# drwangxian/viterbi_spl

Hardware: AMD Instinct MI355X
Metric: Viterbi Mframes/s at S=361 T=30k; achieved HBM GB/s vs peak (higher is better)
Workload: dtype f32

## Files before the change

viterbi_spl_amd/csrc/banded.hip:

```cpp
#include "device_common.hpp"

namespace vit {

template <int W, int NWT, bool DW, bool DBG, int NXT, typename ET>
__global__ void __launch_bounds__((NWT + (DW ? 3 : 2)) * 64) banded_forward_kernel(FwdArgs a) {
    extern __shared__ __align__(16) unsigned char smem[];
    constexpr int NP = NWT * 64;
    constexpr int EPL = NWT;
    const int S = a.S, SP = a.SP, T = a.T, SD = a.SD;
    constexpr int DC = NP + 16;
    float* dls = reinterpret_cast<float*>(smem);
    float* dl = dls + 4;
    float* Pv = dls + 4 * DC;
    float* Sv = Pv + NP + 1;
    float* Dv = Sv + NP + 1;
    VI* tot = reinterpret_cast<VI*>(Dv + kMaxDenseRows);

    const int tid = threadIdx.x;
    const int lane = tid & 63;
    const int wv = __builtin_amdgcn_readfirstlane(tid >> 6);
    const int song = blockIdx.x;
    const int Tb = song_length(a.lengths, song, T);
    const ET* __restrict__ E = reinterpret_cast<const ET*>(a.logE) + (size_t)song * T * S;
    float* __restrict__ hist = a.hist + (size_t)song * T * SD;
// ... 259 lines not shown
    }
    const int sh = a.win_shift;
    const int lov = (tvalid ? lo : S - W) + sh;
    const float* rp = dls + 4 + (lov & 3) * DC + (lov & ~3) + 16 * hh;
    constexpr bool XS = XQ;
    float* fmp = fmg + (XS ? split_fm_slot(lane, is_x) : fm_slot(lane));
    static_assert(!XQ || NXT == 1, "the extra column leaves M by address only where the launcher proved its quad idle");

    for (int k = tid; k < L::reset; k += NW * 64) dls[k] = -INFINITY;
    __syncthreads();

#ifdef VIT_TIMING_HOOKS
    const bool probe = (a.debug & 48) != 0;
    constexpr bool wprobe = WPR;
    WaveProbe wp_;
#else
    constexpr bool probe = false;
#endif
    unsigned long long clk0 = 0ull, rt0 = 0ull;

    auto body = [&](auto role, auto resets) {
        constexpr bool HALF = decltype(role)::value, RESETS = decltype(resets)::value;
        constexpr int WL = HALF ? W / 2 : WF;
        constexpr bool TRIM = WL % 4 != 0;
        const float cj = own ? reinterpret_cast<const float*>(a.image + a.off_rowc)[jc] : -INFINITY;
        float aw[WL];
        float xa[NXL > 0 ? NXL : 1];
        {
            const float* __restrict__ tab = reinterpret_cast<const float*>(a.image + a.off_tabA);
            const float* __restrict__ xaT = reinterpret_cast<const float*>(a.image + a.off_extraA);
#pragma unroll
            for (int w = 0; w < WL; ++w) aw[w] = tvalid ? tab[(size_t)(w + (HALF ? 16 * hh : 0)) * SP + jc] : -INFINITY;
#pragma unroll
            for (int k = 0; k < NXL; ++k)
                xa[k] = (tvalid && k < nx && (!HALF || hh == 1)) ? xaT[(size_t)k * SP + jc] : -INFINITY;
        }
        [[maybe_unused]] float* wp = nullptr;
        if constexpr (HALF) wp = dls + 4 + sh + j + hh * split_upper_off(DC);
        else {
            static_assert(L::dls == 0 && DC == kSplitCopyStride && BUF == 4 * DC, "split_addtid_base / split_addtid_imm (plan.hpp) speak of this layout");
            static_assert(split_addtid_imm(1, 3) + split_addtid_base(3, NWF - 1) + 4 * 64 <= (int)L::bytes() && L::bytes() < 65536,
                          "the largest immediate, the largest base and their sum with the lane term: inside the segment, hence 16 bits each");
            lds_addtid_base(reinterpret_cast<const float*>(smem + split_addtid_base(sh, wv)));
        }
        [[maybe_unused]] int xo[NXL > 0 ? NXL : 1];
        if constexpr (!XS) {
#pragma unroll
            for (int k = 0; k < NXL; ++k) {
                xo[k] = 4 + sh + xcol[k];
                asm volatile("" : "+v"(xo[k]));
            }
        }

        auto produce = [&](const float dn, auto wbc, const int G, const int Z) {
            constexpr int WB = decltype(wbc)::value;
            if constexpr (HALF) {
#pragma unroll
                for (int c = 0; c < 2; ++c) wp[WB * BUF + floor_copy_off(DC, c)] = dn;
            } else {
                split_frames(std::make_integer_sequence<int, 4>{}, [&](auto cc) {
                    static_assert(split_addtid_imm(WB, decltype(cc)::value) == 4 * (WB * BUF + floor_copy_off(DC, decltype(cc)::value)), "the ds_write_b32 form's offset");
                    lds_store_addtid<split_addtid_imm(WB, decltype(cc)::value)>(dn);
                });
            }
            fm_publish(fmp + G * kFmGroupFloats, (!XQ && NXL > 0 && is_x) ? -INFINITY : dn);
            if constexpr (RESETS) fmg[Z * kFmGroupFloats + lane] = -INFINITY;
        };

        {
            const float d0 = tvalid ? reinterpret_cast<const float*>(a.image + a.off_logpi)[j] + load_e<ET>(E + j) : -INFINITY;
            if (own) hist[j] = d0;
            produce(d0, std::integral_constant<int, 0>{}, 0, 1);
        }
        auto frame_barrier = [&] {
            if constexpr (!HALF) __builtin_amdgcn_s_waitcnt(split_waitcnt(kNoVmWait, 0));
            __syncthreads();
        };
        float er[PF];
#pragma unroll
        for (int k = 0; k < PF; ++k) er[k] = load_e<ET>(E + (size_t)(1 + k < Tb ? 1 + k : Tb - 1) * S + jld);
#pragma unroll
        for (int w = 0; w < WL; ++w) asm volatile("" ::"v"(aw[w]));
#pragma unroll
        for (int k = 0; k < NXL; ++k) asm volatile("" ::"v"(xa[k]));
        asm volatile("" ::"v"(cj));
        frame_barrier();

        const unsigned rowH = 4u * (unsigned)SD, rowE = (unsigned)sizeof(ET) * (unsigned)S;
        float* hb = hist;
        const ET* eb = E;
        unsigned elim = 0;
        auto round_bases = [&](const int t) {
            const int r = split_prefetch_row(t, 0, PF, Tb, false);
            const int ahead = Tb - 1 - r < PF ? Tb - 1 - r : PF;
            hb = hist + (size_t)(t - 1) * SD;
            eb = E + (size_t)r * S;
            elim = (unsigned)ahead * rowE;
        };
        auto interior_bases = [&](const int t) {
            hb = hist + (size_t)(t - 1) * SD;
            eb = E + (size_t)split_prefetch_row(t, 0, PF, Tb, true) * S;
        };
        auto frame = [&](float& e_slot, auto uc, auto ic) {
            constexpr int u = decltype(uc)::value;
            constexpr bool INTERIOR = decltype(ic)::value;
            constexpr int RB = u & 1, WB = RB ^ 1;
            const int GR = u % kFmGroups, GW = (u + 1) % kFmGroups, GZ = (u + 2) % kFmGroups;
            const f32x4* __restrict__ win = reinterpret_cast<const f32x4*>(rp + RB * BUF);
            float xd[NXL > 0 ? NXL : 1];
            f32x4 fq;
            [[maybe_unused]] float m0, m1 = -INFINITY, m2 = -INFINITY, m3 = -INFINITY;
            if constexpr (!XS) {
#pragma unroll
                for (int k = 0; k < NXL; ++k) xd[k] = dls[xo[k] + RB * BUF];
            }
            fq = reinterpret_cast<const f32x4*>(fmg + GR * kFmGroupFloats)[0];
            asm volatile("" ::: "memory");
            f32x4 dw[WL / 4];
#pragma unroll
            for (int q = 0; q < WL / 4; ++q) dw[q] = win[q];
            [[maybe_unused]] float ds = 0.f;
            if constexpr (TRIM) ds = (rp + RB * BUF)[WL - 1];
            __builtin_amdgcn_sched_barrier(0);
#ifdef VIT_TIMING_HOOKS
            if constexpr (wprobe && !TRIM) wp_.first_data(fq);
#endif
            if constexpr (TRIM) {
                static_assert(split_reads_behind(WL / 4, 0) == WL / 4 + 1 - 2, "behind the first pair: every other window read of the burst");
                __builtin_amdgcn_s_waitcnt(split_waitcnt(kNoVmWait, split_reads_behind(WL / 4, 0)));
                asm volatile("" : "+v"(fq), "+v"(dw[0]), "+v"(dw[1]));
#ifdef VIT_TIMING_HOOKS
                if constexpr (wprobe) wp_.first_data(fq);
#endif
            }
            const float M = XS ? fmaxf(fmaxf(fq.x, fq.y), fq.z) : fmaxf(fmaxf(fq.x, fq.y), fmaxf(fq.z, fq.w));
            if constexpr (XS) xd[0] = fq.w;
            m0 = M + cj;
            asm volatile("" ::"v"(m0));
            __builtin_amdgcn_sched_barrier(0);
            float mx;
            constexpr int vmw = PF - 1 + u;
            static_assert(vmw <= 2 * (PF - 1) && 2 * (PF - 1) < kNoVmWait, "vmcnt bound: one store and one load per frame, 6-bit field");
            if constexpr (TRIM) {
                constexpr int NQ = WL / 4, TQ = NQ % 2 ? 1 : 2, NPB = (NQ - TQ) / 2;
                static_assert(NXL == 1 && NQ >= 3 && 2 * NPB + TQ == NQ && 4 * NQ + 1 == WL, "pairs of quads, then the tail: one or two quads and one float");
                static_assert(split_reads_behind(NQ, 0) <= 15, "lgkmcnt is a four-bit field");
                static_assert(split_reads_behind(NQ, NPB - 1) == TQ + 1, "behind the last pair stand the tail's reads -- TQ quads and the float -- and nothing else");
                static_assert(split_reads_behind(NQ, NPB) + 2 == TQ + 1 && TQ <= 2, "the tail's wait, lgkmcnt(0), leaves no window read out");
                float mb = xd[0] + xa[0];
                asm volatile("" ::"v"(mb));
                split_frames(std::make_integer_sequence<int, NPB>{}, [&](auto gc) {
                    constexpr int w = 8 * decltype(gc)::value;
                    f32x4 da = dw[w / 4], db = dw[w / 4 + 1];
                    if constexpr (decltype(gc)::value >= 1) {
                        constexpr int behind = split_reads_behind(NQ, decltype(gc)::value);
                        static_assert(behind >= TQ + 1 && behind + 2 == split_reads_behind(NQ, decltype(gc)::value - 1), "two reads fewer than the pair before");
                        __builtin_amdgcn_s_waitcnt(split_waitcnt(kNoVmWait, behind));
                        asm volatile("" : "+v"(da), "+v"(db));
                    }
                    f32x2 c0_ = f32x2{da.x, da.y} + f32x2{aw[w + 0], aw[w + 1]};
                    f32x2 c1_ = f32x2{da.z, da.w} + f32x2{aw[w + 2], aw[w + 3]};
                    f32x2 c2_ = f32x2{db.x, db.y} + f32x2{aw[w + 4], aw[w + 5]};
                    f32x2 c3_ = f32x2{db.z, db.w} + f32x2{aw[w + 6], aw[w + 7]};
                    asm volatile("" : "+v"(c0_), "+v"(c1_), "+v"(c2_), "+v"(c3_));
                    m0 = fmaxf(fmaxf(m0, c0_.x), c0_.y);
                    mb = fmaxf(fmaxf(mb, c1_.x), c1_.y);
                    m0 = fmaxf(fmaxf(m0, c2_.x), c2_.y);
                    mb = fmaxf(fmaxf(mb, c3_.x), c3_.y);
                });
                {
                    constexpr int w = 8 * NPB;
                    f32x4 da = dw[w / 4], db = dw[NQ - 1];
                    __builtin_amdgcn_s_waitcnt(split_waitcnt(vmw, 0));
                    if constexpr (TQ == 2) asm volatile("" : "+v"(da), "+v"(db), "+v"(ds)); else asm volatile("" : "+v"(da), "+v"(ds));
                    f32x2 c0_ = f32x2{da.x, da.y} + f32x2{aw[w + 0], aw[w + 1]};
                    f32x2 c1_ = f32x2{da.z, da.w} + f32x2{aw[w + 2], aw[w + 3]};
                    float cs = ds + aw[WL - 1];
                    if constexpr (TQ == 2) {
                        f32x2 c2_ = f32x2{db.x, db.y} + f32x2{aw[w + 4], aw[w + 5]};
                        f32x2 c3_ = f32x2{db.z, db.w} + f32x2{aw[w + 6], aw[w + 7]};
                        asm volatile("" : "+v"(c0_), "+v"(c1_), "+v"(c2_), "+v"(c3_), "+v"(cs));
                        m0 = fmaxf(fmaxf(m0, c0_.x), c0_.y);
                        mb = fmaxf(fmaxf(mb, c1_.x), c1_.y);
                        m0 = fmaxf(fmaxf(m0, c2_.x), c2_.y);
                        mb = fmaxf(fmaxf(mb, c3_.x), c3_.y);
                    } else {
                        asm volatile("" : "+v"(c0_), "+v"(c1_), "+v"(cs));
                        m0 = fmaxf(fmaxf(m0, c0_.x), c0_.y);
                        mb = fmaxf(fmaxf(mb, c1_.x), c1_.y);
                    }
                    mx = fmaxf(fmaxf(m0, mb), cs);
                }
            } else {
                split_frames(std::make_integer_sequence<int, WL / 8>{}, [&](auto gc) {
                    constexpr int w = 8 * decltype(gc)::value;
                    constexpr bool last = w + 8 == WL;
                    constexpr bool pairw = w + 16 >= WL && w >= 8;
                    f32x4 da = dw[w / 4], db = dw[w / 4 + 1];
                    if constexpr (pairw) {
                        __builtin_amdgcn_s_waitcnt(split_waitcnt(last ? vmw : kNoVmWait, last ? 0 : 2));
                        asm volatile("" : "+v"(da), "+v"(db));
                    }
                    f32x2 c0_ = f32x2{da.x, da.y} + f32x2{aw[w + 0], aw[w + 1]};
                    f32x2 c1_ = f32x2{da.z, da.w} + f32x2{aw[w + 2], aw[w + 3]};
                    f32x2 c2_ = f32x2{db.x, db.y} + f32x2{aw[w + 4], aw[w + 5]};
                    f32x2 c3_ = f32x2{db.z, db.w} + f32x2{aw[w + 6], aw[w + 7]};
                    asm volatile("" : "+v"(c0_), "+v"(c1_), "+v"(c2_), "+v"(c3_));
                    m0 = fmaxf(fmaxf(m0, c0_.x), c0_.y);
                    m1 = fmaxf(fmaxf(m1, c1_.x), c1_.y);
                    m2 = fmaxf(fmaxf(m2, c2_.x), c2_.y);
                    m3 = fmaxf(fmaxf(m3, c3_.x), c3_.y);
                });
#pragma unroll
                for (int k = 0; k < NXL; ++k) m1 = fmaxf(m1, xd[k] + xa[k]);
                mx = fmaxf(fmaxf(m0, m1), fmaxf(m2, m3));
            }
            if constexpr (HALF) mx = max_lane_xor8(mx);
            const float dn = mx + e_slot;
#ifdef VIT_TIMING_HOOKS
            if constexpr (wprobe) wp_.before_publish(dn);
#endif
            const float sv = (HALF && is_fm) ? M : dn;
            const unsigned eso = INTERIOR ? (unsigned)u * rowE : ((unsigned)u * rowE < elim ? (unsigned)u * rowE : elim);
            produce(dn, std::integral_constant<int, WB>{}, GW, GZ);
            asm volatile("" ::: "memory");
            row_store_f32(hb, hoffb, sv, (unsigned)u * rowH);
            e_slot = row_load_e<ET>(eb, eoffb, eso);
#ifdef VIT_TIMING_HOOKS
            if constexpr (wprobe) wp_.barrier(); else
#endif
            frame_barrier();
        };
#ifdef VIT_TIMING_HOOKS
        if constexpr (wprobe) wp_.start();
#endif
        clk0 = probe ? __builtin_amdgcn_s_memtime() : 0ull;
        rt0 = probe ? __builtin_amdgcn_s_memrealtime() : 0ull;
        if constexpr (HALF) __builtin_amdgcn_s_setprio(1);
        int t = 1;
        for (; split_round_interior(t, PF, Tb); t += PF) {
// ... 363 lines not shown
```

viterbi_spl_amd/csrc/banded_floor.inc:

```
__device__ __forceinline__ __amdgpu_buffer_rsrc_t row_rsrc(const void* row) {
    return __builtin_amdgcn_make_buffer_rsrc(const_cast<void*>(row), (short)0, -1, 0x00020000);
}
__device__ __forceinline__ void row_store_f32(float* row, unsigned off, float v, unsigned soff = 0) {
    __builtin_amdgcn_raw_buffer_store_b32(__float_as_uint(v), row_rsrc(row), off, soff, 0);
}
template <typename ET>
__device__ __forceinline__ float row_load_e(const ET* row, unsigned off, unsigned soff = 0);
template <>
__device__ __forceinline__ float row_load_e<float>(const float* row, unsigned off, unsigned soff) {
    return __uint_as_float(__builtin_amdgcn_raw_buffer_load_b32(row_rsrc(row), off, soff, 0));
}
template <>
__device__ __forceinline__ float row_load_e<__half>(const __half* row, unsigned off, unsigned soff) {
    return __half2float(__ushort_as_half(__builtin_amdgcn_raw_buffer_load_b16(row_rsrc(row), off, soff, 0)));
}

inline constexpr int kFmGroups = 4;
inline constexpr int kFmGroupFloats = 64;
inline constexpr int kFmSlots = 4;
__device__ __forceinline__ int fm_slot(int lane) { return 4 * (lane & 3) + ((lane >> 2) & 3); }
__device__ __forceinline__ void fm_publish(float* slot, float v) {
    v = fmaxf(v, __int_as_float(__builtin_amdgcn_update_dpp(0, __float_as_int(v), 0xb1, 0xf, 0xf, false)));
    v = fmaxf(v, __int_as_float(__builtin_amdgcn_update_dpp(0, __float_as_int(v), 0x4e, 0xf, 0xf, false)));
    __hip_atomic_fetch_max(slot, v, __ATOMIC_RELAXED, __HIP_MEMORY_SCOPE_WORKGROUP);
// ... 2 lines not shown
#ifdef VIT_TIMING_HOOKS
struct WaveProbe {
    unsigned long long t_rel = 0, t_pub = 0, t_dat = 0, work = 0, wait = 0, data = 0;
    __device__ __forceinline__ void start() { t_rel = t_dat = __builtin_amdgcn_s_memtime(); }
    template <typename V>
    __device__ __forceinline__ void first_data(V& first) {
        asm volatile("" : "+v"(first));
        __builtin_amdgcn_sched_barrier(0);
        t_dat = __builtin_amdgcn_s_memtime();
        __builtin_amdgcn_sched_barrier(0);
    }
    __device__ __forceinline__ void before_publish(float dn) {
        __builtin_amdgcn_sched_barrier(0);
        asm volatile("" ::"v"(dn));
        t_pub = __builtin_amdgcn_s_memtime();
        __builtin_amdgcn_sched_barrier(0);
    }
    __device__ __forceinline__ void barrier() {
        unsigned long long t_in, t_out;
        asm volatile("s_waitcnt lgkmcnt(0)\n\ts_memtime %0\n\ts_barrier\n\ts_memtime %1\n\ts_waitcnt lgkmcnt(0)"
                     : "=&s"(t_in), "=&s"(t_out) : "s"(t_pub), "s"(t_dat) : "memory");
        work += t_pub - t_rel;
        data += t_dat - t_rel;
        wait += t_out - t_in;
        t_rel = t_dat = t_out;
    }
    __device__ __forceinline__ void finish(float* scratch, int wv, int lane, int frames) const {
        if (lane != 0) return;
        const float n = (float)(frames > 0 ? frames : 1);
        scratch[4 * wv + 0] = (float)__builtin_amdgcn_s_getreg((1 << 11) | (4 << 6) | 4);
        scratch[4 * wv + 1] = (float)work / n;
        scratch[4 * wv + 2] = (float)wait / n;
        scratch[4 * wv + 3] = n;
        scratch[48 + wv] = (float)data / n;
    }
};
#endif

template <int W, int NWT, WgVariant V = WgVariant::Plain>
struct FloorLds {
    static constexpr int NP = NWT * 64;
    static constexpr int DC = NP + 16;
    static constexpr int BUF = 4 * DC;
    static constexpr int WR = (W == 128 && NWT > 8) ? (V != WgVariant::Plain ? 88 : 96) : W;
    static constexpr int dls = 0;
    static constexpr int fmg = dls + 2 * BUF;
    static constexpr int reset = fmg + kFmGroups * kFmGroupFloats;
    static constexpr int tot = reset;
    static constexpr int awl = tot + 16 * (int)(sizeof(VI) / sizeof(float));
    static constexpr int end = awl + (W - WR) / 4 * 4 * NP;
    static_assert(sizeof(float) * end <= kLdsBytes, "one workgroup's LDS");
    static constexpr size_t bytes() { return sizeof(float) * end; }
};
constexpr int floor_copy_off(int DC, int c) { return c * DC - c; }
constexpr int split_upper_off(int DC) { return floor_copy_off(DC, 2); }
inline constexpr int kSplitFullWaves = 4, kSplitHalfWaves = 4;
inline constexpr int kSplitStates = 64 * kSplitFullWaves + 32 * kSplitHalfWaves;
using FloorSplitLds = FloorLds<32, kSplitStates / 64>;
constexpr int split_half_of(int lane) { return (lane >> 3) & 1; }
constexpr int split_half_target(int lane) { return ((lane >> 4) << 3) | (lane & 7); }
inline constexpr int kSplitXSlot = 3;
constexpr int split_fm_slot(int lane, bool is_x) { return 4 * (lane & 3) + (is_x ? kSplitXSlot : (lane >> 2) % 3); }

template <int W, int NWT, int NXT, int PF, typename ET, WgVariant V = WgVariant::Plain, bool WPR = false>
__global__ void __launch_bounds__(NWT * 64) banded_floor_forward_kernel(FwdArgs a) {
    static_assert(!WPR || V == WgVariant::Plain, "the per-wave probe exists for the plain kernel only");
    using L = FloorLds<W, NWT, V>;
    constexpr bool PK = V == WgVariant::Packed, CK = V == WgVariant::Ckpt, PC = V == WgVariant::PackedCkpt;
    constexpr bool PKx = PK || PC;
    constexpr bool CKx = CK || PC;
    extern __shared__ __align__(16) unsigned char smem[];
    constexpr int NP = L::NP, DC = L::DC, BUF = L::BUF, WR = L::WR;
    float* dls = reinterpret_cast<float*>(smem) + L::dls;
    float* fmg = dls + L::fmg;
    VI* tot = reinterpret_cast<VI*>(dls + L::tot);
    f32x4* awl = reinterpret_cast<f32x4*>(dls + L::awl);
    const int S = a.S, SP = a.SP, T = a.T, SD = a.SD;
    constexpr bool GEN = NXT < 0;
    constexpr int NXL = GEN ? kMaxExtras : NXT;
    const int nx = GEN ? a.n_extras : NXT;

    const int tid = threadIdx.x;
    const int lane = tid & 63;
    const int wv = __builtin_amdgcn_readfirstlane(tid >> 6);
    constexpr int kPast = 1, kRowBias = 1;
#define VIT_WG_CURSOR 1
#include "wg_cursor.inc"
#define VIT_WG_CURSOR 2
#include "wg_cursor.inc"

    const int j = tid;
    const bool tvalid = j < S;
    const int jc = tvalid ? j : 0;
    const int jld = tvalid ? j : S - 1;
    const unsigned hoff = tvalid ? (unsigned)(SD + j) : ((j == S && !(CKx && ck_every > 0)) ? (unsigned)S : (unsigned)(SD + S + 1));
    const bool is_fm = j == S;
    const unsigned hoffb = 4u * hoff, eoffb = (unsigned)(sizeof(ET) * jld);
    const int lo = reinterpret_cast<const int32_t*>(a.image + a.off_lo)[jc];
    const float cj = tvalid ? reinterpret_cast<const float*>(a.image + a.off_rowc)[jc] : -INFINITY;
    float aw[WR];
    float xa[NXL > 0 ? NXL : 1];
    int xcol[NXL > 0 ? NXL : 1];
    bool is_x = false;
    {
        const float* __restrict__ tab = reinterpret_cast<const float*>(a.image + a.off_tabA);
        const float* __restrict__ xaT = reinterpret_cast<const float*>(a.image + a.off_extraA);
#pragma unroll
        for (int w = 0; w < WR; ++w) aw[w] = tvalid ? tab[(size_t)w * SP + jc] : -INFINITY;
#pragma unroll
        for (int q = 0; q < (W - WR) / 4; ++q) {
            f32x4 wv4;
            wv4.x = tvalid ? tab[(size_t)(WR + 4 * q + 0) * SP + jc] : -INFINITY;
            wv4.y = tvalid ? tab[(size_t)(WR + 4 * q + 1) * SP + jc] : -INFINITY;
            wv4.z = tvalid ? tab[(size_t)(WR + 4 * q + 2) * SP + jc] : -INFINITY;
            wv4.w = tvalid ? tab[(size_t)(WR + 4 * q + 3) * SP + jc] : -INFINITY;
// ... 255 lines not shown
```

viterbi_spl_amd/csrc/device_common.hpp:

```cpp
#pragma once
#include <hip/hip_fp16.h>
#include <hip/hip_runtime.h>

#include <cstddef>
#include <cstdint>
#include <type_traits>

#include "kernels.hpp"

namespace vit {

inline constexpr int kBig = 0x7fffffff;
inline constexpr size_t kLdsBytes = 160 * 1024;

typedef float f32x2 __attribute__((ext_vector_type(2)));
typedef float f32x4 __attribute__((ext_vector_type(4)));
typedef float f32x4_u __attribute__((ext_vector_type(4), aligned(4)));
typedef float f32x2_u __attribute__((ext_vector_type(2), aligned(4)));
typedef int i32x4_u __attribute__((ext_vector_type(4), aligned(4)));
typedef _Float16 f16x2_u __attribute__((ext_vector_type(2), aligned(2)));
typedef _Float16 f16x4_u __attribute__((ext_vector_type(4), aligned(2)));

__device__ __forceinline__ int song_length(const int64_t* lengths, int song, int T) {
    if (!lengths) return T;
// ... 27 lines not shown
        "s_nop 1\n\t"
        "v_max_f32_dpp %0, %0, %0 row_bcast:15 row_mask:0xa bank_mask:0xf\n\t"
        "s_nop 1\n\t"
        "v_max_f32_dpp %0, %0, %0 row_bcast:31 row_mask:0xc bank_mask:0xf\n\t"
        "s_nop 1"
        : "+v"(x));
    return x;
}
__device__ __forceinline__ float wave_max_all(float x) {
    return __int_as_float(__builtin_amdgcn_readlane(__float_as_int(wave_scan_max(x)), 63));
}
template <int CTRL, int ROW_MASK>
__device__ __forceinline__ double dpp_max_step_f64(const double x) {
    const long long b = __double_as_longlong(x);
    const int lo = (int)(unsigned)(b & 0xffffffffll), hi = (int)(b >> 32);
    const int slo = __builtin_amdgcn_update_dpp(lo, lo, CTRL, ROW_MASK, 0xf, false);
    const int shi = __builtin_amdgcn_update_dpp(hi, hi, CTRL, ROW_MASK, 0xf, false);
    const double s = __longlong_as_double(((long long)shi << 32) | (long long)(unsigned)slo);
    return fmax(x, s);
}
__device__ __forceinline__ double wave_scan_max_f64(double x) {
    x = dpp_max_step_f64<0x111, 0xf>(x);
    x = dpp_max_step_f64<0x112, 0xf>(x);
    x = dpp_max_step_f64<0x114, 0xf>(x);
    x = dpp_max_step_f64<0x118, 0xf>(x);
    x = dpp_max_step_f64<0x142, 0xa>(x);
    x = dpp_max_step_f64<0x143, 0xc>(x);
    return x;
}
__device__ __forceinline__ double readlane_f64(const double x, const int l) {
    const long long b = __double_as_longlong(x);
    const unsigned lo = (unsigned)__builtin_amdgcn_readlane((int)(unsigned)(b & 0xffffffffll), l);
    const unsigned hi = (unsigned)__builtin_amdgcn_readlane((int)(b >> 32), l);
    return __longlong_as_double((long long)(((unsigned long long)hi << 32) | lo));
}
__device__ __forceinline__ double wave_max_all_f64(const double x) { return readlane_f64(wave_scan_max_f64(x), 63); }
__device__ __forceinline__ float max_other_half(float x) {
    const auto r = __builtin_amdgcn_permlane32_swap(__float_as_uint(x), __float_as_uint(x), false, false);
    return fmaxf(__uint_as_float(r[0]), __uint_as_float(r[1]));
}
inline constexpr int kDppRowRor8 = 0x128;
__device__ __forceinline__ float max_lane_xor8(float x) {
    return fmaxf(x, __int_as_float(__builtin_amdgcn_update_dpp(0, __float_as_int(x), kDppRowRor8, 0xf, 0xf, false)));
}
__device__ __forceinline__ void lds_addtid_base(const float* p) {
    const unsigned base = (unsigned)(unsigned long)(__attribute__((address_space(3))) const float*)p;
    asm volatile("s_mov_b32 m0, %0\n\ts_nop 0" ::"s"(base) : "memory");
}
template <int BYTE_OFF>
__device__ __forceinline__ void lds_store_addtid(float v) {
    static_assert(BYTE_OFF >= 0 && BYTE_OFF < 65536 && BYTE_OFF % 4 == 0, "the instruction's 16-bit offset field");
    asm volatile("ds_write_addtid_b32 %0 offset:%1" ::"v"(v), "n"(BYTE_OFF) : "memory");
}
__device__ __forceinline__ float wave_shift_up(float x, float fill) {
    return __int_as_float(__builtin_amdgcn_update_dpp(__float_as_int(fill), __float_as_int(x), 0x138, 0xf, 0xf, false));
}
__device__ __forceinline__ float wave_shift_down(float x, float fill) {
    return __int_as_float(__builtin_amdgcn_update_dpp(__float_as_int(fill), __float_as_int(x), 0x130, 0xf, 0xf, false));
}
__device__ __forceinline__ float dpp_shr1(float x) {
    return __int_as_float(__builtin_amdgcn_update_dpp(0, __float_as_int(x), 0x138, 0xf, 0xf, true));
}
__device__ __forceinline__ float dpp_shl1(float x) {
    return __int_as_float(__builtin_amdgcn_update_dpp(0, __float_as_int(x), 0x130, 0xf, 0xf, true));
}

struct VI {
    float v;
    int i;
};

__device__ __forceinline__ VI vi_identity() { return VI{-INFINITY, kBig}; }
__device__ __forceinline__ VI op_fwd(VI earlier, VI later) { return later.v > earlier.v ? later : earlier; }
__device__ __forceinline__ VI op_rev(VI acc, VI next) { return next.v >= acc.v ? next : acc; }

template <int CTRL, int ROW_MASK>
__device__ __forceinline__ VI dpp_fetch(VI x) {
    VI r;
    r.v = __int_as_float(__builtin_amdgcn_update_dpp(__float_as_int(-INFINITY), __float_as_int(x.v), CTRL,
                                                     ROW_MASK, 0xf, false));
    r.i = __builtin_amdgcn_update_dpp(kBig, x.i, CTRL, ROW_MASK, 0xf, false);
    return r;
}

template <bool REV>
__device__ __forceinline__ VI wave_scan(VI x) {
#define VIT_SCAN_STEP(CTRL, MASK)                        \
    {                                                    \
        VI s = dpp_fetch<CTRL, MASK>(x);                 \
        x = REV ? op_rev(s, x) : op_fwd(s, x);           \
    }
    VIT_SCAN_STEP(0x111, 0xf)
    VIT_SCAN_STEP(0x112, 0xf)
    VIT_SCAN_STEP(0x114, 0xf)
    VIT_SCAN_STEP(0x118, 0xf)
    VIT_SCAN_STEP(0x142, 0xa)
    VIT_SCAN_STEP(0x143, 0xc)
#undef VIT_SCAN_STEP
    return x;
}

__device__ __forceinline__ void terminal_argmax(float dj, int j, bool valid, VI* tot, int nw, int32_t* last_state,
                                                float* loglik, int song) {
    VI x{valid ? dj : -INFINITY, valid ? j : kBig};
    x = wave_scan<false>(x);
    if ((threadIdx.x & 63) == 63) tot[threadIdx.x >> 6] = x;
// ... 27 lines not shown
```

viterbi_spl_amd/csrc/floor_lds_check.hip:

```cpp
#include <cstdio>
#include <cstdlib>
#include <vector>

#include "device_common.hpp"

namespace vit {
#include "banded_floor.inc"
}
using namespace vit;

static int failures = 0;
#define CHECK(cond, ...)                                                     \
    do {                                                                     \
        if (!(cond)) {                                                       \
            if (++failures <= 20) { std::printf("FAIL %s: ", #cond); std::printf(__VA_ARGS__); std::printf("\n"); } \
        }                                                                    \
    } while (0)

static bool write2_encodable(int stride) { return stride >= 0 && stride <= 255; }
static bool write2st64_encodable(int stride) { return stride >= 0 && stride % 64 == 0 && stride / 64 <= 255; }

struct Segment {
    std::vector<int> owner;
    explicit Segment(int n) : owner((size_t)n, -1) {}
// ... 151 lines not shown
            was[hw] = half_wave_read_cycles(S, off, sh, hw, old_half_of, old_half_target);
            now[hw] = half_wave_read_cycles(S, off, sh, hw, split_half_of, split_half_target);
            if (sh == off % 4) CHECK(now[hw] <= was[hw], "S %d sh %d half wave %d: %d LDS cycles for its window reads, %d with the halves 32 lanes apart", S, sh, hw, now[hw], was[hw]);
        }
        std::printf("split window reads S %d off %d sh %d%s: ds_read_b128 cycles per half wave, halves 32 lanes apart %d / %d / %d / %d, partner l ^ 8 %d / %d / %d / %d\n",
                    S, off, sh, sh == off % 4 ? " (the plan's)" : "", was[0], was[1], was[2], was[3], now[0], now[1], now[2], now[3]);
    }
}

static void replay_slot_map() {
    int cases = 0;
    for (int S = 64 * kSplitFullWaves + 1; S < kSplitStates; S += 4) {
        const int x = S - 1;
        CHECK(x % 4 == 0, "x %d", x);
        bool x_reached = false;
        for (int wv = 0; wv < kSplitFullWaves + kSplitHalfWaves; ++wv) {
            bool quad_in_m[16] = {};
            for (int lane = 0; lane < 64; ++lane) {
                const bool half = wv >= kSplitFullWaves;
                const int j = half ? 64 * kSplitFullWaves + 32 * (wv - kSplitFullWaves) + split_half_target(lane) : 64 * wv + lane;
                const int slot = split_fm_slot(lane, j == x);
                CHECK(slot >= 0 && slot < 16, "slot %d", slot);
                bool quad_has_x = false;
                for (int m = 0; m < 4; ++m) {
                    const int lm = (lane & ~3) | m;
                    const int jm = half ? 64 * kSplitFullWaves + 32 * (wv - kSplitFullWaves) + split_half_target(lm) : 64 * wv + lm;
                    quad_has_x |= jm == x;
                    if (quad_has_x && jm != x) CHECK(jm >= S, "S %d: state %d shares a quad with x and is live", S, jm);
                }
                if (slot < kSplitXSlot) {
                    CHECK(!quad_has_x, "S %d wave %d lane %d: a quad that holds x adds into M slot %d", S, wv, lane, slot);
                    quad_in_m[lane >> 2] = true;
                }
                if (slot == kSplitXSlot) {
                    CHECK(j == x, "S %d wave %d lane %d (state %d) adds into the extra column's slot", S, wv, lane, j);
                    x_reached = true;
                }
            }
            for (int q = 0; q < 16; ++q) {
                bool has_x = false;
                for (int m = 0; m < 4; ++m) {
                    const int lm = 4 * q + m;
                    has_x |= (wv >= kSplitFullWaves ? 64 * kSplitFullWaves + 32 * (wv - kSplitFullWaves) + split_half_target(lm) : 64 * wv + lm) == x;
                }
                CHECK(quad_in_m[q] != has_x, "S %d wave %d quad %d: %s", S, wv, q, has_x ? "holds x and reaches M" : "reaches none of slots 0 .. 2");
            }
        }
        CHECK(x_reached, "S %d: no lane adds x into slot %d", S, kSplitXSlot);
        ++cases;
    }
    std::printf("split slot map: every quad without x reaches one of slots 0 .. 2, x reaches slot %d alone: ok (%d state counts)\n", kSplitXSlot, cases);
}

template <int W, int NWT>
static void replay_pair() {
    char name[64];
    std::snprintf(name, sizeof name, "FloorLds<%d, %d>", W, NWT);
    replay<FloorLds<W, NWT, WgVariant::Plain>, W>(name, NWT, false);
    if constexpr (W == 128 && NWT > 8) {
        std::snprintf(name, sizeof name, "FloorLds<%d, %d, Packed>", W, NWT);
        replay<FloorLds<W, NWT, WgVariant::Packed>, W>(name, NWT, false);
    }
}
template <int W>
static void replay_width() {
    replay_pair<W, 2>();
    replay_pair<W, 4>();
    replay_pair<W, 6>();
    replay_pair<W, 8>();
    replay_pair<W, 12>();
}

int main() {
    static_assert(sizeof(kBandedWidths) / sizeof(int) == 6, "one call per instantiated window width");
    replay_width<16>();
    replay_width<32>();
    replay_width<64>();
    replay_width<84>();
    replay_width<96>();
    replay_width<128>();
    replay<FloorSplitLds, 32>("FloorSplitLds (split kernel)", kSplitStates / 64, true);
    replay_lane_map();
    replay_slot_map();
    replay_read_cycles(361, 15);
    replay_read_cycles(321, 13);
    static_assert(2 * FloorSplitLds::bytes() <= kLdsBytes && 2 * FloorLds<32, 6>::bytes() <= kLdsBytes, "two workgroups share a CU's LDS");
    if (failures) { std::printf("%d check(s) failed\n", failures); return 1; }
    std::printf("floor LDS layouts: all checks passed\n");
    return 0;
}
```

viterbi_spl_amd/csrc/plan.hpp:

```cpp
#pragma once
#include <cstddef>
#include <cstdint>
#include <vector>

namespace vit {

constexpr int kMaxExtras = 4;
constexpr int kMaxDenseRows = 4;
inline constexpr int kBandedWidths[] = {16, 32, 64, 84, 96, 128};
constexpr bool banded_width_instantiated(int W) {
    for (int w : kBandedWidths)
        if (w == W) return true;
    return false;
}

struct BandedPlan {
    bool ok = false;
    int S = 0;
    int SP = 0;
    float c0 = 0.f;
    std::vector<float> rowc;
    int n_extras = 0;
    int extras[kMaxExtras] = {0, 0, 0, 0};
    int n_dense = 0;
// ... 3 lines not shown
    std::vector<int32_t> lo;
    std::vector<int32_t> kind;
    bool lo_affine = false;
    bool floor_ok = false;
    std::vector<int32_t> live_last;
    bool pair_ok = false;
    std::vector<int32_t> lo2;
    bool lo2_affine = false;
    int lo2_off = 0;
    int lo_off = 0;

    bool step_ok = false;
    int step_bw = 0, step_kb = 0;
    std::vector<float> stepC;
    float step_cn = 0.f;

    bool floor_all_ok = false;
    bool wave_ok = false;
    int wave_npl = 0;
    int wave_d = 0;
    int wave_dk = 0;
};

constexpr int kWaveMaxExtras = 2;
constexpr int wave_table_d(int npl, int d) { return (npl == 6 && d <= 14) ? 14 : 0; }
constexpr int wave_pairs(int dk) { return dk + 1; }
constexpr int wave_halo(int npl, int dk) { return (dk + npl - 1) / npl; }
constexpr int wave_p0e(int npl, int dk, int k) { return (k + npl * wave_halo(npl, dk) - dk) & ~1; }

constexpr int kMaxStepBands = 15;
void analyze_step(const float* logA_T, int S, BandedPlan& bp);

BandedPlan analyze_banded(const float* logA_T, int S);
int floor_live_width(const BandedPlan& bp, int n_rows);
constexpr int kSplitFullRows = 256;
inline constexpr int kSplitLiveWidths[] = {25, 29};
constexpr int split_full_width(int live, int W, int S, int n_extras, bool f16) {
    if (W != 32 || S <= kSplitFullRows || S >= 384 || n_extras != 1 || f16) return W;
    for (int w : kSplitLiveWidths)
        if (live >= 1 && live <= w && w < W) return w;
    return W;
}
constexpr bool split_round_full(int t, int PF, int Tb) { return t + PF - 1 <= Tb - 1; }
constexpr bool split_round_interior(int t, int PF, int Tb) { return t + 2 * PF - 1 <= Tb - 1; }
constexpr int split_prefetch_row(int t, int u, int PF, int Tb, bool interior) {
    const int r = t + u + PF;
    return interior || r < Tb - 1 ? r : Tb - 1;
}
inline constexpr int kSplitPrefetch = 12;
inline constexpr int kSplitCopyStride = 384 + 16;
constexpr int split_copy_pos(int sh, int j, int b, int c) { return 4 + sh + j + b * 4 * kSplitCopyStride + c * kSplitCopyStride - c; }
constexpr int split_addtid_base(int sh, int wave) { return 4 * (4 + sh + 64 * wave); }
constexpr int split_addtid_imm(int b, int c) { return 4 * (b * 4 * kSplitCopyStride + c * kSplitCopyStride - c); }

struct ImageLayout {
    int S = 0, SP = 0, S4 = 0, W = 0, n_extras = 0, n_dense = 0;
    size_t off_logpi = 0;
    size_t off_A4 = 0;
    size_t off_lo = 0;
    size_t off_kind = 0;
    size_t off_tabA = 0;
    size_t off_extraA = 0;
    size_t off_denseA = 0;
    size_t off_Arow = 0;
    size_t off_rowc = 0;
    size_t off_lo2 = 0;
    size_t off_tabP = 0;
    size_t off_tabX = 0;
    size_t off_stepC = 0;
    size_t off_tabV = 0;
    size_t bytes = 0;
};

struct PackedCkptSchedule {
    std::vector<int32_t> unit_song, unit_seg;
    std::vector<int64_t> launch_begin, ckpt_base;
};
int64_t packed_ckpt_units(const int64_t* offsets, int64_t B, int64_t K);
void packed_ckpt_schedule(const int64_t* offsets, int64_t B, int64_t K, int64_t max_units, PackedCkptSchedule& out);

bool packed_chunk_table(const int64_t* offsets, int64_t B, int64_t streams, int64_t max_chunks, int64_t min_frames, bool round_nearest,
                        int64_t capacity, int32_t* chunk_base, int32_t* wave_song, int64_t* largest);

ImageLayout make_layout(int S, const BandedPlan& bp);
void fill_image(const float* logA_T, const float* log_pi, const BandedPlan& bp,
                const ImageLayout& L, uint8_t* image);

}
```

viterbi_spl_amd/csrc/plan_host_capi.cpp:

```cpp
#include <cstring>
#include <vector>

#include "plan.hpp"

extern "C" {

struct vph_plan {
    vit::BandedPlan bp;
    vit::ImageLayout L;
    std::vector<uint8_t> image;
};

vph_plan* vph_create(const float* logA_T, const float* log_pi, int S) {
    vph_plan* p = new vph_plan();
    p->bp = vit::analyze_banded(logA_T, S);
    if (!p->bp.ok) vit::analyze_step(logA_T, S, p->bp);
    p->L = vit::make_layout(S, p->bp);
    p->image.resize(p->L.bytes);
    vit::fill_image(logA_T, log_pi, p->bp, p->L, p->image.data());
    return p;
}
void vph_destroy(vph_plan* p) { delete p; }

void vph_info(const vph_plan* p, int* info, float* c0) {
    info[0] = p->bp.ok; info[1] = p->bp.S; info[2] = p->bp.SP; info[3] = p->bp.W;
    info[4] = p->bp.n_extras; info[5] = p->bp.n_dense; info[6] = p->bp.max_window;
    for (int k = 0; k < 4; ++k) { info[7 + k] = p->bp.extras[k]; info[11 + k] = p->bp.dense_rows[k]; }
    info[15] = p->L.S4 | (p->bp.pair_ok ? 0x10000 : 0) | (p->bp.floor_ok ? 0x20000 : 0) | (p->bp.step_ok ? 0x40000 : 0) |
               ((p->bp.step_ok ? p->bp.step_kb : 0) << 20) | ((p->bp.step_ok ? p->bp.step_bw : 0) << 24);
    *c0 = p->bp.c0;
}
void vph_offsets(const vph_plan* p, long long* off) {
    off[0] = p->L.off_logpi; off[1] = p->L.off_A4; off[2] = p->L.off_lo; off[3] = p->L.off_kind;
    off[4] = p->L.off_tabA; off[5] = p->L.off_extraA; off[6] = p->L.off_denseA; off[7] = p->L.bytes;
    off[8] = p->L.off_Arow; off[9] = p->L.off_rowc; off[10] = p->L.off_lo2; off[11] = p->L.off_tabP;
}
void vph_wave(const vph_plan* p, long long* w) {
    w[0] = p->bp.wave_ok; w[1] = p->bp.wave_npl; w[2] = p->bp.wave_d; w[3] = p->bp.wave_dk;
    w[4] = p->bp.floor_all_ok; w[5] = (long long)p->L.off_tabV;
}
void vph_step(const vph_plan* p, long long* s, float* cn) {
    s[0] = p->bp.step_ok; s[1] = p->bp.step_ok ? p->bp.step_bw : 0; s[2] = p->bp.step_ok ? p->bp.step_kb : 0;
    s[3] = (long long)p->L.off_stepC;
    *cn = p->bp.step_ok ? p->bp.step_cn : 0.f;
}
int vph_live_width(const vph_plan* p, int n_rows) { return vit::floor_live_width(p->bp, n_rows); }
int vph_split_full_width(const vph_plan* p, int f16) {
    return vit::split_full_width(vit::floor_live_width(p->bp, vit::kSplitFullRows), p->bp.W, p->bp.S, p->bp.ok ? p->bp.n_extras : 0, f16 != 0);
}
int vph_split_rounds(int Tb, int pf, int* frame, int* row, int* cls, int cap) {
    const int PF = pf > 0 ? pf : vit::kSplitPrefetch;
    if (Tb < 1 || PF % 2 != 0) return -1;
    int n = 0;
    auto emit = [&](int t, int u, int c) {
        if (n < cap) { frame[n] = t + u; row[n] = vit::split_prefetch_row(t, u, PF, Tb, c == 2); cls[n] = c; }
        ++n;
    };
    int t = 1;
    for (; vit::split_round_interior(t, PF, Tb); t += PF)
        for (int u = 0; u < PF; ++u) emit(t, u, 2);
    for (; vit::split_round_full(t, PF, Tb); t += PF)
        for (int u = 0; u < PF; ++u) emit(t, u, 1);
    for (int u = 0; u < PF - 1; ++u)
        if (t + u < Tb) emit(t, u, 0);
    return n <= cap ? n : -1;
}
int vph_split_prefetch(void) { return vit::kSplitPrefetch; }
int vph_split_addtid(int sh, int wave, int lane, int b, int c, int* out) {
    if (sh < 0 || sh > 3 || wave < 0 || wave >= vit::kSplitFullRows / 64 || lane < 0 || lane > 63 || b < 0 || b > 1 || c < 0 || c > 3) return -1;
    out[0] = vit::split_addtid_base(sh, wave);
    out[1] = vit::split_addtid_imm(b, c);
    out[2] = vit::split_copy_pos(sh, 64 * wave + lane, b, c);
    return 0;
}
void vph_image(const vph_plan* p, unsigned char* out) { std::memcpy(out, p->image.data(), p->image.size()); }

long long vph_packed_ckpt_schedule(const long long* offsets, long long B, long long K, long long max_units, int* unit_song, int* unit_seg,
                                   long long cap_units, long long* launch_begin, long long cap_launches, long long* ckpt_base) {
    std::vector<int64_t> off(offsets, offsets + B + 1);
    const int64_t units = vit::packed_ckpt_units(off.data(), B, K);
    if (units < 0 || units > cap_units) return -1;
    vit::PackedCkptSchedule sc;
    vit::packed_ckpt_schedule(off.data(), B, K, max_units, sc);
    const long long nl = (long long)sc.launch_begin.size() - 1;
    if (nl > cap_launches) return -1;
    for (size_t u = 0; u < sc.unit_song.size(); ++u) { unit_song[u] = sc.unit_song[u]; unit_seg[u] = sc.unit_seg[u]; }
    for (size_t l = 0; l < sc.launch_begin.size(); ++l) launch_begin[l] = sc.launch_begin[l];
    for (size_t b = 0; b < sc.ckpt_base.size(); ++b) ckpt_base[b] = sc.ckpt_base[b];
    return nl;
}

int vph_packed_chunk_table(const long long* offsets, long long B, long long streams, long long max_chunks, long long min_frames, int round_nearest,
                           long long capacity, int* chunk_base, int* wave_song, long long* largest) {
    std::vector<int64_t> off(offsets, offsets + B + 1);
    int64_t big = 0;
    const bool ok = vit::packed_chunk_table(off.data(), B, streams, max_chunks, min_frames, round_nearest != 0, capacity, chunk_base, wave_song, &big);
    *largest = big;
    return ok ? 1 : 0;
}

}
```

Measured before the change: 532.5.

## Quad-reduce produced values with DPP before publishing via LDS atomic max

In the split full-wave path the four add-tid copy stores are emitted in one asm block, interleaved with two DPP max steps that reduce each quad of lanes. The reduced value is then published with a workgroup-scope atomic max instead of the prior fm_publish, which should cut the number of lanes contending on each slot. The trimmed max loop also defers initialising the x accumulator and loosens the register pin on the first partial so the scheduler has more freedom. Host-side LDS bank-conflict replay helpers and checks are added, and the layout constants move to plan.hpp. The atomic path is correct only if slot resets and the quad-to-slot mapping still agree with the consumer.

```diff
diff --git a/viterbi_spl_amd/csrc/banded.hip b/viterbi_spl_amd/csrc/banded.hip
--- a/viterbi_spl_amd/csrc/banded.hip
+++ b/viterbi_spl_amd/csrc/banded.hip
@@ -335,8 +335,15 @@
             }
         }
 
+        constexpr bool QUADASM = !HALF && (XQ || NXL == 0);
         auto produce = [&](const float dn, auto wbc, const int G, const int Z) {
             constexpr int WB = decltype(wbc)::value;
+            if constexpr (QUADASM) {
+                const float q = lds_store_addtid4_quad_max<split_addtid_imm(WB, 0), split_addtid_imm(WB, 1), split_addtid_imm(WB, 2),
+                                                           split_addtid_imm(WB, 3)>(dn);
+                __hip_atomic_fetch_max(fmp + G * kFmGroupFloats, q, __ATOMIC_RELAXED, __HIP_MEMORY_SCOPE_WORKGROUP);
+                return;
+            }
             if constexpr (HALF) {
 #pragma unroll
                 for (int c = 0; c < 2; ++c) wp[WB * BUF + floor_copy_off(DC, c)] = dn;
@@ -430,8 +437,7 @@
                 static_assert(split_reads_behind(NQ, 0) <= 15, "lgkmcnt is a four-bit field");
                 static_assert(split_reads_behind(NQ, NPB - 1) == TQ + 1, "behind the last pair stand the tail's reads -- TQ quads and the float -- and nothing else");
                 static_assert(split_reads_behind(NQ, NPB) + 2 == TQ + 1 && TQ <= 2, "the tail's wait, lgkmcnt(0), leaves no window read out");
-                float mb = xd[0] + xa[0];
-                asm volatile("" ::"v"(mb));
+                float mb;
                 split_frames(std::make_integer_sequence<int, NPB>{}, [&](auto gc) {
                     constexpr int w = 8 * decltype(gc)::value;
                     f32x4 da = dw[w / 4], db = dw[w / 4 + 1];
@@ -445,6 +451,10 @@
                     f32x2 c1_ = f32x2{da.z, da.w} + f32x2{aw[w + 2], aw[w + 3]};
                     f32x2 c2_ = f32x2{db.x, db.y} + f32x2{aw[w + 4], aw[w + 5]};
                     f32x2 c3_ = f32x2{db.z, db.w} + f32x2{aw[w + 6], aw[w + 7]};
+                    if constexpr (decltype(gc)::value == 0) {
+                        mb = xd[0] + xa[0];
+                        asm volatile("" : "+v"(c0_), "+v"(c1_), "+v"(c2_), "+v"(c3_) : "v"(mb));
+                    } else
                     asm volatile("" : "+v"(c0_), "+v"(c1_), "+v"(c2_), "+v"(c3_));
                     m0 = fmaxf(fmaxf(m0, c0_.x), c0_.y);
                     mb = fmaxf(fmaxf(mb, c1_.x), c1_.y);
@@ -462,13 +472,13 @@
                     if constexpr (TQ == 2) {
                         f32x2 c2_ = f32x2{db.x, db.y} + f32x2{aw[w + 4], aw[w + 5]};
                         f32x2 c3_ = f32x2{db.z, db.w} + f32x2{aw[w + 6], aw[w + 7]};
-                        asm volatile("" : "+v"(c0_), "+v"(c1_), "+v"(c2_), "+v"(c3_), "+v"(cs));
+                        asm volatile("" : "+v"(c1_), "+v"(c2_), "+v"(c3_), "+v"(cs) : "v"(c0_));
                         m0 = fmaxf(fmaxf(m0, c0_.x), c0_.y);
                         mb = fmaxf(fmaxf(mb, c1_.x), c1_.y);
                         m0 = fmaxf(fmaxf(m0, c2_.x), c2_.y);
                         mb = fmaxf(fmaxf(mb, c3_.x), c3_.y);
                     } else {
-                        asm volatile("" : "+v"(c0_), "+v"(c1_), "+v"(cs));
+                        asm volatile("" : "+v"(c1_), "+v"(cs) : "v"(c0_));
                         m0 = fmaxf(fmaxf(m0, c0_.x), c0_.y);
                         mb = fmaxf(fmaxf(mb, c1_.x), c1_.y);
                     }
diff --git a/viterbi_spl_amd/csrc/banded_floor.inc b/viterbi_spl_amd/csrc/banded_floor.inc
--- a/viterbi_spl_amd/csrc/banded_floor.inc
+++ b/viterbi_spl_amd/csrc/banded_floor.inc
@@ -78,15 +78,8 @@
     static_assert(sizeof(float) * end <= kLdsBytes, "one workgroup's LDS");
     static constexpr size_t bytes() { return sizeof(float) * end; }
 };
-constexpr int floor_copy_off(int DC, int c) { return c * DC - c; }
-constexpr int split_upper_off(int DC) { return floor_copy_off(DC, 2); }
-inline constexpr int kSplitFullWaves = 4, kSplitHalfWaves = 4;
-inline constexpr int kSplitStates = 64 * kSplitFullWaves + 32 * kSplitHalfWaves;
 using FloorSplitLds = FloorLds<32, kSplitStates / 64>;
-constexpr int split_half_of(int lane) { return (lane >> 3) & 1; }
-constexpr int split_half_target(int lane) { return ((lane >> 4) << 3) | (lane & 7); }
-inline constexpr int kSplitXSlot = 3;
-constexpr int split_fm_slot(int lane, bool is_x) { return 4 * (lane & 3) + (is_x ? kSplitXSlot : (lane >> 2) % 3); }
+static_assert(FloorSplitLds::DC == kSplitCopyStride && FloorSplitLds::fmg == kSplitSlotGroups, "plan.hpp replays this layout");
 
 template <int W, int NWT, int NXT, int PF, typename ET, WgVariant V = WgVariant::Plain, bool WPR = false>
 __global__ void __launch_bounds__(NWT * 64) banded_floor_forward_kernel(FwdArgs a) {
diff --git a/viterbi_spl_amd/csrc/device_common.hpp b/viterbi_spl_amd/csrc/device_common.hpp
--- a/viterbi_spl_amd/csrc/device_common.hpp
+++ b/viterbi_spl_amd/csrc/device_common.hpp
@@ -103,6 +103,18 @@
     static_assert(BYTE_OFF >= 0 && BYTE_OFF < 65536 && BYTE_OFF % 4 == 0, "the instruction's 16-bit offset field");
     asm volatile("ds_write_addtid_b32 %0 offset:%1" ::"v"(v), "n"(BYTE_OFF) : "memory");
 }
+template <int O0, int O1, int O2, int O3>
+__device__ __forceinline__ float lds_store_addtid4_quad_max(float v) {
+    static_assert(O0 >= 0 && O1 >= 0 && O2 >= 0 && O3 >= 0 && O0 < 65536 && O1 < 65536 && O2 < 65536 && O3 < 65536 &&
+                  (O0 | O1 | O2 | O3) % 4 == 0, "the instruction's 16-bit offset field");
+    float q;
+    asm volatile("ds_write_addtid_b32 %1 offset:%2\n\tds_write_addtid_b32 %1 offset:%3\n\t"
+                 "v_max_f32_dpp %0, %1, %1 quad_perm:[1,0,3,2] row_mask:0xf bank_mask:0xf bound_ctrl:1\n\t"
+                 "ds_write_addtid_b32 %1 offset:%4\n\tds_write_addtid_b32 %1 offset:%5\n\t"
+                 "v_max_f32_dpp %0, %0, %0 quad_perm:[2,3,0,1] row_mask:0xf bank_mask:0xf bound_ctrl:1"
+                 : "=&v"(q) : "v"(v), "n"(O0), "n"(O1), "n"(O2), "n"(O3) : "memory");
+    return q;
+}
 __device__ __forceinline__ float wave_shift_up(float x, float fill) {
     return __int_as_float(__builtin_amdgcn_update_dpp(__float_as_int(fill), __float_as_int(x), 0x138, 0xf, 0xf, false));
 }
diff --git a/viterbi_spl_amd/csrc/floor_lds_check.hip b/viterbi_spl_amd/csrc/floor_lds_check.hip
--- a/viterbi_spl_amd/csrc/floor_lds_check.hip
+++ b/viterbi_spl_amd/csrc/floor_lds_check.hip
@@ -227,6 +227,34 @@
     std::printf("split slot map: every quad without x reaches one of slots 0 .. 2, x reaches slot %d alone: ok (%d state counts)\n", kSplitXSlot, cases);
 }
 
+static void replay_conflicts(int S, int off, int WF) {
+    static const int pairs[4][2][2] = {{{0, 1}, {2, 3}}, {{2, 3}, {0, 1}}, {{0, 2}, {1, 3}}, {{1, 3}, {0, 2}}};
+    static const char* kind[6] = {"slot quad read", "window b128", "window b32", "copy writes", "ds_max_f32", "slot reset"};
+    const auto slot = [](int lane, bool is_x) { return split_fm_slot(lane, is_x); };
+    int frame_total[4][2] = {};
+    for (int as = 0; as < 4; ++as)
+        for (int ser = 0; ser < 2; ++ser)
+            for (int rb = 0; rb < 2; ++rb)
+                for (int wv = 0; wv < kSplitFullWaves + kSplitHalfWaves; ++wv) {
+                    int c[6];
+                    split_lds_conflicts(S, off, WF, wv, rb, ser != 0, [&](int half, int k) { return pairs[as][half][k]; }, slot, c);
+                    for (int k = 0; k < 6; ++k) frame_total[as][ser] += c[k];
+                    if (as == 0 && ser == 1 && (rb == 0 || wv == 0))
+                        std::printf("split conflicts S %d WF %d buffer %d wave %d (%s):", S, WF, rb, wv, wv < kSplitFullWaves ? "full" : wv == 7 ? "half, resets" : "half");
+                    if (as == 0 && ser == 1 && (rb == 0 || wv == 0)) {
+                        for (int k = 0; k < 6; ++k) std::printf(" %s %d", kind[k], c[k]);
+                        std::printf("\n");
+                    }
+                    CHECK(c[0] == 0 && c[5] == 0, "S %d wave %d: the broadcast slot read and the linear reset must be conflict-free", S, wv);
+                    if (wv < kSplitFullWaves) CHECK(c[3] == 0, "S %d wave %d: the add-tid stores are linear in the lane", S, wv);
+                }
+    for (int as = 0; as < 4; ++as) {
+        std::printf("split conflicts S %d WF %d, half-wave copies lower (%d, %d) upper (%d, %d)%s: %.3f extra LDS cycles per wave-frame, %.3f with the ds_max_f32 lanes of one address serialised\n",
+                    S, WF, pairs[as][0][0], pairs[as][0][1], pairs[as][1][0], pairs[as][1][1], as == 0 ? " (the kernel's)" : "", frame_total[as][0] / 16.0, frame_total[as][1] / 16.0);
+        CHECK(frame_total[as][0] >= frame_total[0][0] && frame_total[as][1] >= frame_total[0][1], "S %d: copy assignment %d has fewer conflict cycles than the kernel's", S, as);
+    }
+}
+
 template <int W, int NWT>
 static void replay_pair() {
     char name[64];
@@ -259,6 +287,9 @@
     replay_slot_map();
     replay_read_cycles(361, 15);
     replay_read_cycles(321, 13);
+    replay_conflicts(361, 15, 29);
+    replay_conflicts(321, 13, 25);
+    replay_conflicts(361, 15, 32);
     static_assert(2 * FloorSplitLds::bytes() <= kLdsBytes && 2 * FloorLds<32, 6>::bytes() <= kLdsBytes, "two workgroups share a CU's LDS");
     if (failures) { std::printf("%d check(s) failed\n", failures); return 1; }
     std::printf("floor LDS layouts: all checks passed\n");
diff --git a/viterbi_spl_amd/csrc/plan.hpp b/viterbi_spl_amd/csrc/plan.hpp
--- a/viterbi_spl_amd/csrc/plan.hpp
+++ b/viterbi_spl_amd/csrc/plan.hpp
@@ -79,6 +79,79 @@
 constexpr int split_copy_pos(int sh, int j, int b, int c) { return 4 + sh + j + b * 4 * kSplitCopyStride + c * kSplitCopyStride - c; }
 constexpr int split_addtid_base(int sh, int wave) { return 4 * (4 + sh + 64 * wave); }
 constexpr int split_addtid_imm(int b, int c) { return 4 * (b * 4 * kSplitCopyStride + c * kSplitCopyStride - c); }
+constexpr int floor_copy_off(int DC, int c) { return c * DC - c; }
+constexpr int split_upper_off(int DC) { return floor_copy_off(DC, 2); }
+inline constexpr int kSplitFullWaves = 4, kSplitHalfWaves = 4;
+inline constexpr int kSplitStates = 64 * kSplitFullWaves + 32 * kSplitHalfWaves;
+inline constexpr int kSplitSlotGroups = 2 * 4 * kSplitCopyStride;
+constexpr int split_half_of(int lane) { return (lane >> 3) & 1; }
+constexpr int split_half_target(int lane) { return ((lane >> 4) << 3) | (lane & 7); }
+inline constexpr int kSplitXSlot = 3;
+constexpr int split_fm_slot(int lane, bool is_x) { return 4 * (lane & 3) + (is_x ? kSplitXSlot : (lane >> 2) % 3); }
+constexpr int split_lane_target(int wave, int lane) {
+    return wave < kSplitFullWaves ? 64 * wave + lane : 64 * kSplitFullWaves + 32 * (wave - kSplitFullWaves) + split_half_target(lane);
+}
+constexpr int split_window_pos(int S, int off, int sh, int wave, int lane, int rb) {
+    const int j = split_lane_target(wave, lane);
+    const int lo = j - off < 0 ? 0 : (j - off > S - 32 ? S - 32 : j - off);
+    const int lov = (j < S ? lo : S - 32) + sh;
+    return 4 + (lov & 3) * kSplitCopyStride + (lov & ~3) + (wave >= kSplitFullWaves ? 16 * split_half_of(lane) : 0) + rb * 4 * kSplitCopyStride;
+}
+inline int lds_extra_cycles(const int* pos, const int (*groups)[16], int ngroups, int per_group, int width, int banks, bool same_address_serialises) {
+    int total = 0;
+    for (int g = 0; g < ngroups; ++g) {
+        int worst = 1;
+        for (int bank = 0; bank < banks; ++bank) {
+            int seen[64], n = 0, lanes = 0;
+            for (int i = 0; i < per_group; ++i) {
+                const int lane = groups ? groups[g][i] : g * per_group + i;
+                for (int k = 0; k < width; ++k) {
+                    const int a = pos[lane] + k;
+                    if (a % banks != bank) continue;
+                    ++lanes;
+                    bool dup = false;
+                    for (int q = 0; q < n; ++q) dup |= seen[q] == a;
+                    if (!dup) seen[n++] = a;
+                }
+            }
+            const int ways = same_address_serialises ? lanes : n;
+            if (ways > worst) worst = ways;
+        }
+        total += worst - 1;
+    }
+    return total;
+}
+inline constexpr int kLdsReadB128Groups[4][16] = {{0, 1, 2, 3, 12, 13, 14, 15, 20, 21, 22, 23, 24, 25, 26, 27},
+                                                  {4, 5, 6, 7, 8, 9, 10, 11, 16, 17, 18, 19, 28, 29, 30, 31},
+                                                  {32, 33, 34, 35, 44, 45, 46, 47, 52, 53, 54, 55, 56, 57, 58, 59},
+                                                  {36, 37, 38, 39, 40, 41, 42, 43, 48, 49, 50, 51, 60, 61, 62, 63}};
+template <typename CopyOf, typename SlotOf>
+inline void split_lds_conflicts(int S, int off, int WF, int wave, int rb, bool atomics_serialise, CopyOf copy_of, SlotOf slot_of, int out[6]) {
+    const int sh = off % 4, wb = rb ^ 1, x = S - 1;
+    const bool hw = wave >= kSplitFullWaves;
+    int pos[64];
+    for (int k = 0; k < 6; ++k) out[k] = 0;
+    for (int l = 0; l < 64; ++l) pos[l] = kSplitSlotGroups;
+    out[0] = lds_extra_cycles(pos, kLdsReadB128Groups, 4, 16, 4, 64, false);
+    for (int q = 0; q < (hw ? 4 : WF / 4); ++q) {
+        for (int l = 0; l < 64; ++l) pos[l] = split_window_pos(S, off, sh, wave, l, rb) + 4 * q;
+        out[1] += lds_extra_cycles(pos, kLdsReadB128Groups, 4, 16, 4, 64, false);
+    }
+    if (!hw && WF % 4) {
+        for (int l = 0; l < 64; ++l) pos[l] = split_window_pos(S, off, sh, wave, l, rb) + WF - 1;
+        out[2] = lds_extra_cycles(pos, nullptr, 2, 32, 1, 32, false);
+    }
+    for (int k = 0; k < (hw ? 2 : 4); ++k) {
+        for (int l = 0; l < 64; ++l) pos[l] = split_copy_pos(sh, split_lane_target(wave, l), wb, hw ? copy_of(split_half_of(l), k) : k);
+        out[3] += lds_extra_cycles(pos, nullptr, 2, 32, 1, 32, false);
+    }
+    for (int l = 0; l < 64; ++l) pos[l] = kSplitSlotGroups + slot_of(l, split_lane_target(wave, l) == x);
+    out[4] = lds_extra_cycles(pos, nullptr, 2, 32, 1, 32, atomics_serialise);
+    if (wave == kSplitFullWaves + kSplitHalfWaves - 1) {
+        for (int l = 0; l < 64; ++l) pos[l] = kSplitSlotGroups + 64 + l;
+        out[5] = lds_extra_cycles(pos, nullptr, 2, 32, 1, 32, false);
+    }
+}
 
 struct ImageLayout {
     int S = 0, SP = 0, S4 = 0, W = 0, n_extras = 0, n_dense = 0;
diff --git a/viterbi_spl_amd/csrc/plan_host_capi.cpp b/viterbi_spl_amd/csrc/plan_host_capi.cpp
--- a/viterbi_spl_amd/csrc/plan_host_capi.cpp
+++ b/viterbi_spl_amd/csrc/plan_host_capi.cpp
@@ -73,6 +73,28 @@
     out[2] = vit::split_copy_pos(sh, 64 * wave + lane, b, c);
     return 0;
 }
+int vph_split_lds_conflicts(int S, int off, int WF, int wave, int rb, int atomics_serialise, int assignment, int* out) {
+    if (S <= vit::kSplitFullRows || S >= vit::kSplitStates || off < 0 || off > 31 || (WF != 25 && WF != 29 && WF != 32) || wave < 0 ||
+        wave >= vit::kSplitFullWaves + vit::kSplitHalfWaves || rb < 0 || rb > 1 || assignment < 0 || assignment > 3)
+        return -1;
+    static const int pairs[4][2][2] = {{{0, 1}, {2, 3}}, {{2, 3}, {0, 1}}, {{0, 2}, {1, 3}}, {{1, 3}, {0, 2}}};
+    vit::split_lds_conflicts(S, off, WF, wave, rb, atomics_serialise != 0, [&](int half, int k) { return pairs[assignment][half][k]; },
+                             [](int lane, bool is_x) { return vit::split_fm_slot(lane, is_x); }, out);
+    return 0;
+}
+int vph_split_maps(int S, int off, int wave, int lane, int b, int* out) {
+    if (S <= vit::kSplitFullRows || S >= vit::kSplitStates || off < 0 || off > 31 || wave < 0 || wave >= 8 || lane < 0 || lane > 63 || b < 0 || b > 1) return -1;
+    const bool hw = wave >= vit::kSplitFullWaves;
+    const int sh = off % 4, j = vit::split_lane_target(wave, lane), hh = hw ? vit::split_half_of(lane) : 0;
+    out[0] = j; out[1] = hh; out[2] = vit::split_fm_slot(lane, false); out[3] = vit::split_fm_slot(lane, true);
+    for (int k = 0; k < 4; ++k) {
+        out[4 + k] = -1;
+        if (!hw) out[4 + k] = vit::split_copy_pos(sh, j, b, k);
+        else if (k < 2) out[4 + k] = 4 + sh + j + hh * vit::split_upper_off(vit::kSplitCopyStride) + b * 4 * vit::kSplitCopyStride + vit::floor_copy_off(vit::kSplitCopyStride, k);
+    }
+    out[8] = vit::split_window_pos(S, off, sh, wave, lane, b);
+    return 0;
+}
 void vph_image(const vph_plan* p, unsigned char* out) { std::memcpy(out, p->image.data(), p->image.size()); }
 
 long long vph_packed_ckpt_schedule(const long long* offsets, long long B, long long K, long long max_units, int* unit_song, int* unit_seg,
```

After: 542.5, median of 6. 1.9% higher.
